# Aatrick/LightDiffusion

Hardware: AMD Instinct MI355X
Metric: UNet denoise steps/sec at 512x512 (higher is better)
Workload: dtype f16 (fp32 accumulate); 1 GPU; SD1.5 512x512 UNet CFG step, euler_ancestral / normal-30, batch 8/GPU (UNet batch 16), latent 64x64; global_batch=8, parallelism=dp1 (replicas, RCCL cond broadcast), hip_graph=True, setup_before_warmup=hipGraph capture + one untimed schedule pass per workload

## Files before the change

### include/ld_mi355x.h

```cpp
#ifndef LD_MI355X_H
#define LD_MI355X_H

#include <stddef.h>
#include <stdint.h>

#ifdef __cplusplus
extern "C" {
#endif

#define LD_OK 0
#define LD_ERR_ARG 1
#define LD_ERR_SHAPE 2
#define LD_ERR_HIP 3
#define LD_ERR_STATE 4

#define LD_F16 0
#define LD_F32 1

const char* ld_version(void);
const char* ld_status_string(int status);

typedef struct {
    int in_channels, out_channels, model_channels;
    int num_levels;
// ... 59 lines not shown

typedef struct {
    int in_nc, out_nc;
    int nf, gc;
    int nb;
    int scale;
} ld_esrgan_config;

typedef struct ld_esrgan ld_esrgan;

int ld_esrgan_create(const ld_esrgan_config* cfg, ld_esrgan** out);
void ld_esrgan_destroy(ld_esrgan* e);
int ld_esrgan_param_count(const ld_esrgan* e);
int ld_esrgan_param_info(const ld_esrgan* e, int index, const char** name, int* ndim, int64_t shape[4]);
int ld_esrgan_load_param(ld_esrgan* e, const char* name, const void* dev_src, int dtype, void* stream);
int ld_esrgan_reserve(ld_esrgan* e, int max_b, int max_h, int max_w);
size_t ld_esrgan_workspace_bytes(const ld_esrgan* e);
size_t ld_esrgan_plan_bytes(ld_esrgan* e, int b, int h, int w);
int ld_esrgan_forward(ld_esrgan* e, const float* x, float* out, int b, int h, int w, void* stream);
int ld_esrgan_profile(ld_esrgan* e, const float* x, float* out, int b, int h, int w, void* stream);
int ld_esrgan_profile_launches(const ld_esrgan* e, char* buf, size_t buf_bytes);
int ld_esrgan_last_launches(const ld_esrgan* e);
double ld_esrgan_last_flops(const ld_esrgan* e);

int ld_op_linear(const void* x, const void* w, const void* bias, const void* residual, void* y, int M, int N, int K,
                 float alpha, int act, void* ws, size_t ws_bytes, void* stream);
int ld_op_conv(const void* x1, int c1, const void* x2, int c2, int n, int h, int w, int hv, int wv, int stride, int ksize,
               const void* wt, const void* bias, const void* rowvec, const void* residual, void* y, int cout,
               void* ws, size_t ws_bytes, void* stream);
size_t ld_op_groupnorm_conv_ws_bytes(int c1, int c2, int n, int h, int w, int cout);
int ld_op_groupnorm_conv(const void* x1, int c1, const void* x2, int c2, int n, int h, int w, const void* gamma, const void* beta, float eps,
                         const void* wt, const void* bias, const void* rowvec, const void* residual, void* y, int cout, void* ws,
                         size_t ws_bytes, void* stream);
int ld_op_repack_conv(const void* src_oihw, int dtype, int cout, int cin, void* dst, void* stream);
size_t ld_op_conv_skip_ws_bytes(int c, int sc1, int sc2, int cout);
int ld_op_conv_skip(const void* x, int c, int n, int h, int w, const void* wt, const void* bias, const void* s1, int sc1, const void* s2, int sc2,
                    const void* wskip, const void* bskip, const void* rowvec, void* y, int cout, void* ws, size_t ws_bytes, void* stream);
size_t ld_op_groupnorm_conv_skip_ws_bytes(int c, int sc1, int sc2, int cout, int n, int h, int w);
int ld_op_groupnorm_conv_skip(const void* x, int c, int n, int h, int w, const void* gamma, const void* beta, float eps, const void* wt, const void* bias,
                              const void* s1, int sc1, const void* s2, int sc2, const void* wskip, const void* bskip, const void* rowvec, void* y, int cout,
                              float* part, int* chunks, void* ws, size_t ws_bytes, void* stream);
int ld_op_upconv2x_fold(const void* wt, int cout, int cin, void* wfold, void* stream);
int ld_op_upconv2x(const void* x, int c, int n, int h, int w, int hv, int wv, const void* wt, const void* wfold, const void* bias, void* y, int cout,
                   void* ws, size_t ws_bytes, void* stream);
size_t ld_op_conv_gn_partials_floats(int n, int hw);
int ld_op_conv_gn_partials(const void* x, int c, int n, int h, int w, int hv, int wv, const void* wt, const void* bias,
                           const void* residual, void* y, int cout, float* part, int* chunks, void* ws, size_t ws_bytes, void* stream);
size_t ld_op_groupnorm_ws_bytes(int n, int hw);
int ld_op_groupnorm(const void* x1, int c1, const void* x2, int c2, int n, int hw, const void* gamma, const void* beta,
                    float eps, int silu, void* y, void* ws, void* stream);
int ld_op_layernorm(const void* x, const void* gamma, const void* beta, void* y, int rows, int c, float eps, void* stream);
int ld_op_attention(const void* q, int ldq, const void* k, int ldk, const void* vt, int ldvt, void* o, int ldo, int b,
                    int heads, int lq, int lk, int d, float scale, int causal, void* stream);
int ld_op_attention_rowv(const void* q, int ldq, const void* k, int ldk, const void* v, int ldv, void* o, int ldo, int b,
                         int heads, int lq, int lk, int d, float scale, int causal, void* stream);
int ld_op_softmax_rows(void* s, int rows, int cols, void* stream);
int ld_op_timestep_embed(const float* sigma, const float* log_sigmas, int n_sigmas, int n, int dim, void* out_f16, float* t_out,
                         void* stream);
int ld_op_cfg_combine(const float* den2, float* out, float cfg, size_t n_half, void* stream);
int ld_op_axpby(float* x, float a, const float* y, float b, const float* z, float c, size_t n, void* stream);
int ld_op_hook_check(const void* a, const void* b, size_t words_ab, const void* x, size_t half_words_x, const void* sigma, int half_sigma,
                     int* flags, int epoch, void* stream);

int ld_op_linear_ln(const void* x, const void* w_prod, const void* b_prod, const void* gamma, const void* beta, const void* w,
                    const void* bias, void* t_out, void* y, int M, int C, int N, float eps, void* ws, size_t ws_bytes, void* stream);
int ld_op_linear_ln_geglu(const void* x, const void* w_prod, const void* b_prod, const void* gamma, const void* beta, const void* w,
                          const void* bias, void* t_out, void* y, int M, int C, int N, float eps, void* ws, size_t ws_bytes, void* stream);
int ld_op_bislerp(const float* x, float* tmp, float* y, int n, int c, int h, int w, int h_new, int w_new, void* stream);
int ld_op_esrgan_conv(const void* x, int ldx, int cin, int n, int h, int w, int up, const void* wt, const void* bias, void* y, int ldy, int c_off, int cout,
                      float slope, const void* r1, int ldr1, float s1, const void* r2, int ldr2, float s2, void* stream);
int ld_op_tile_blend(const float* ps, const float* my, const float* mx, int th, int tw, float* out, float* div, int oh, int ow, int y0, int x0, int c,
                     void* stream);
const char* ld_op_last_kernel(void);
int ld_op_lora_merge(const void* base_f16, void* dst_f16, int rows, int cols, const ld_lora_term* terms, int n_terms, void* stream);

int ld_op_u8_resample(const void* src, int src_pitch, int in_w, int in_h, int channels, void* dst, int dst_pitch, int out_w, int out_h, const int* hcoef,
                      int hk, const int* vcoef, int vk, void* tmp, void* stream);
size_t ld_op_u8_resample_tmp_bytes(int in_h, int out_w, int channels);
int ld_op_u8_box_weights(float radius, int* box_radius, unsigned* ww, unsigned* fw);
size_t ld_op_u8_blur_tmp_bytes(int w, int h);
int ld_op_u8_gaussian_blur(const void* src, int src_pitch, void* dst, int dst_pitch, int w, int h, float radius, void* tmp, void* stream);
int ld_op_u8_mask(void* dst, int dst_pitch, int w, int h, int px, int py, int pw, int ph, const void* pattern, int pattern_pitch, void* stream);
int ld_op_u8_composite(void* canvas, int canvas_pitch, int cw, int ch, const void* tile, int tile_pitch, const void* alpha, int alpha_pitch, int x0, int y0,
                       int w, int h, int channels, void* stream);
int ld_op_u8_from_f32(const float* x, void* y, size_t n, void* stream);
int ld_op_f32_from_u8(const void* x, float* y, size_t n, void* stream);

#ifdef __cplusplus
}
#endif
#endif
```

### lightdiffusion_amd/_lib.py

```python
from __future__ import annotations

import ctypes as C
import os

_HERE = os.path.dirname(os.path.abspath(__file__))
LIB_PATH = os.environ.get("LD_MI355X_LIB") or os.path.join(_HERE, "libld_mi355x.so")

OK, ERR_ARG, ERR_SHAPE, ERR_HIP, ERR_STATE = 0, 1, 2, 3, 4
F16, F32 = 0, 1


class UNetConfig(C.Structure):
    _fields_ = [("in_channels", C.c_int), ("out_channels", C.c_int), ("model_channels", C.c_int), ("num_levels", C.c_int),
                ("channel_mult", C.c_int * 8), ("num_res_blocks", C.c_int * 8), ("transformer_depth", C.c_int * 16),
                ("transformer_depth_output", C.c_int * 24), ("transformer_depth_middle", C.c_int),
                ("context_dim", C.c_int), ("num_heads", C.c_int)]


class VAEConfig(C.Structure):
    _fields_ = [("z_channels", C.c_int), ("ch", C.c_int), ("num_levels", C.c_int), ("ch_mult", C.c_int * 8),
                ("num_res_blocks", C.c_int), ("out_ch", C.c_int), ("with_encoder", C.c_int)]


class ESRGANConfig(C.Structure):
# ... 31 lines not shown
    "ld_unet_profile_pair": (_I, [_P, _P, _P, _P, _I, _I, _I, _P, C.POINTER(C.c_double), C.POINTER(C.c_double), C.POINTER(_I)]),
    "ld_unet_profile": (_I, [_P, _P, _P, _P, _I, _I, _I, _P, C.POINTER(C.c_double), C.POINTER(C.c_double), C.POINTER(_I)]),
    "ld_unet_profile_kernels": (_I, [_P, C.c_char_p, _Z]),
    "ld_unet_profile_launches": (_I, [_P, C.c_char_p, _Z]),
    "ld_unet_patch_param": (_I, [_P, C.c_char_p, C.POINTER(LoraTerm), _I, _P]),
    "ld_unet_unpatch": (_I, [_P, C.c_char_p, _P]),
    "ld_unet_read_param": (_I, [_P, C.c_char_p, _P, _P]),
    "ld_unet_refresh_derived": (_I, [_P, _P]),
    "ld_unet_patch_bytes": (_Z, [_P]),
    "ld_unet_last_launches": (_I, [_P]),
    "ld_unet_last_flops": (C.c_double, [_P]),
    "ld_vae_create": (_I, [C.POINTER(VAEConfig), C.POINTER(_P)]),
    "ld_vae_destroy": (None, [_P]),
    "ld_vae_param_count": (_I, [_P]),
    "ld_vae_param_info": (_I, [_P, _I, C.POINTER(C.c_char_p), C.POINTER(_I), C.POINTER(C.c_int64)]),
    "ld_vae_load_param": (_I, [_P, C.c_char_p, _P, _I, _P]),
    "ld_vae_reserve": (_I, [_P, _I, _I, _I]),
    "ld_vae_workspace_bytes": (_Z, [_P]),
    "ld_vae_plan_bytes": (_Z, [_P, _I, _I, _I]),
    "ld_vae_decode": (_I, [_P, _P, _P, _I, _I, _I, _P]),
    "ld_vae_encode": (_I, [_P, _P, _P, _I, _I, _I, _P]),
    "ld_vae_profile": (_I, [_P, _P, _P, _I, _I, _I, _P]),
    "ld_vae_profile_launches": (_I, [_P, C.c_char_p, _Z]),
    "ld_vae_last_launches": (_I, [_P]),
    "ld_vae_last_flops": (C.c_double, [_P]),
    "ld_esrgan_create": (_I, [C.POINTER(ESRGANConfig), C.POINTER(_P)]),
    "ld_esrgan_destroy": (None, [_P]),
    "ld_esrgan_param_count": (_I, [_P]),
    "ld_esrgan_param_info": (_I, [_P, _I, C.POINTER(C.c_char_p), C.POINTER(_I), C.POINTER(C.c_int64)]),
    "ld_esrgan_load_param": (_I, [_P, C.c_char_p, _P, _I, _P]),
    "ld_esrgan_reserve": (_I, [_P, _I, _I, _I]),
    "ld_esrgan_workspace_bytes": (_Z, [_P]),
    "ld_esrgan_plan_bytes": (_Z, [_P, _I, _I, _I]),
    "ld_esrgan_forward": (_I, [_P, _P, _P, _I, _I, _I, _P]),
    "ld_esrgan_profile": (_I, [_P, _P, _P, _I, _I, _I, _P]),
    "ld_esrgan_profile_launches": (_I, [_P, C.c_char_p, _Z]),
    "ld_esrgan_last_launches": (_I, [_P]),
    "ld_esrgan_last_flops": (C.c_double, [_P]),
    "ld_op_linear": (_I, [_P, _P, _P, _P, _P, _I, _I, _I, _F, _I, _P, _Z, _P]),
    "ld_op_conv": (_I, [_P, _I, _P, _I, _I, _I, _I, _I, _I, _I, _I, _P, _P, _P, _P, _P, _I, _P, _Z, _P]),
    "ld_op_groupnorm_conv_ws_bytes": (_Z, [_I, _I, _I, _I, _I, _I]),
    "ld_op_groupnorm_conv": (_I, [_P, _I, _P, _I, _I, _I, _I, _P, _P, _F, _P, _P, _P, _P, _P, _I, _P, _Z, _P]),
    "ld_op_repack_conv": (_I, [_P, _I, _I, _I, _P, _P]),
    "ld_op_upconv2x_fold": (_I, [_P, _I, _I, _P, _P]),
    "ld_op_upconv2x": (_I, [_P, _I, _I, _I, _I, _I, _I, _P, _P, _P, _P, _I, _P, _Z, _P]),
    "ld_op_conv_skip_ws_bytes": (_Z, [_I, _I, _I, _I]),
    "ld_op_conv_skip": (_I, [_P, _I, _I, _I, _I, _P, _P, _P, _I, _P, _I, _P, _P, _P, _P, _I, _P, _Z, _P]),
    "ld_op_groupnorm_conv_skip_ws_bytes": (_Z, [_I, _I, _I, _I, _I, _I, _I]),
    "ld_op_groupnorm_conv_skip": (_I, [_P, _I, _I, _I, _I, _P, _P, _F, _P, _P, _P, _I, _P, _I, _P, _P, _P, _P, _I, _P, _P, _P, _Z, _P]),
    "ld_op_groupnorm_ws_bytes": (_Z, [_I, _I]),
    "ld_op_groupnorm": (_I, [_P, _I, _P, _I, _I, _I, _P, _P, _F, _I, _P, _P, _P]),
    "ld_op_layernorm": (_I, [_P, _P, _P, _P, _I, _I, _F, _P]),
    "ld_op_attention": (_I, [_P, _I, _P, _I, _P, _I, _P, _I, _I, _I, _I, _I, _I, _F, _I, _P]),
    "ld_op_conv_gn_partials_floats": (_Z, [_I, _I]),
    "ld_op_conv_gn_partials": (_I, [_P, _I, _I, _I, _I, _I, _I, _P, _P, _P, _P, _I, _P, _P, _P, _Z, _P]),
    "ld_op_attention_rowv": (_I, [_P, _I, _P, _I, _P, _I, _P, _I, _I, _I, _I, _I, _I, _F, _I, _P]),
    "ld_op_softmax_rows": (_I, [_P, _I, _I, _P]),
    "ld_op_timestep_embed": (_I, [_P, _P, _I, _I, _I, _P, _P, _P]),
    "ld_op_cfg_combine": (_I, [_P, _P, _F, _Z, _P]),
    "ld_op_axpby": (_I, [_P, _F, _P, _F, _P, _F, _Z, _P]),
    "ld_op_hook_check": (_I, [_P, _P, _Z, _P, _Z, _P, _I, _P, _I, _P]),
    "ld_op_linear_ln": (_I, [_P, _P, _P, _P, _P, _P, _P, _P, _P, _I, _I, _I, _F, _P, _Z, _P]),
    "ld_op_linear_ln_geglu": (_I, [_P, _P, _P, _P, _P, _P, _P, _P, _P, _I, _I, _I, _F, _P, _Z, _P]),
    "ld_op_bislerp": (_I, [_P, _P, _P, _I, _I, _I, _I, _I, _I, _P]),
    "ld_op_esrgan_conv": (_I, [_P, _I, _I, _I, _I, _I, _I, _P, _P, _P, _I, _I, _I, _F, _P, _I, _F, _P, _I, _F, _P]),
    "ld_op_tile_blend": (_I, [_P, _P, _P, _I, _I, _P, _P, _I, _I, _I, _I, _I, _P]),
    "ld_op_last_kernel": (C.c_char_p, []),
    "ld_op_lora_merge": (_I, [_P, _P, _I, _I, C.POINTER(LoraTerm), _I, _P]),
    "ld_op_u8_resample": (_I, [_P, _I, _I, _I, _I, _P, _I, _I, _I, _P, _I, _P, _I, _P, _P]),
    "ld_op_u8_resample_tmp_bytes": (_Z, [_I, _I, _I]),
    "ld_op_u8_box_weights": (_I, [_F, C.POINTER(_I), C.POINTER(C.c_uint), C.POINTER(C.c_uint)]),
    "ld_op_u8_blur_tmp_bytes": (_Z, [_I, _I]),
    "ld_op_u8_gaussian_blur": (_I, [_P, _I, _P, _I, _I, _I, _F, _P, _P]),
    "ld_op_u8_mask": (_I, [_P, _I, _I, _I, _I, _I, _I, _I, _P, _I, _P]),
    "ld_op_u8_composite": (_I, [_P, _I, _I, _I, _P, _I, _P, _I, _I, _I, _I, _I, _I, _P]),
    "ld_op_u8_from_f32": (_I, [_P, _P, _Z, _P]),
    "ld_op_f32_from_u8": (_I, [_P, _P, _Z, _P]),
}


def lib() -> C.CDLL:
    global _lib
    if _lib is None:
        if not os.path.exists(LIB_PATH):
            raise ImportError(f"{LIB_PATH} not found — build it with `python -c 'import __graft_entry__ as g; g.build()'` "
                              f"or `make -C lightdiffusion_amd/csrc`.  There is no CPU / PyTorch fallback for the hot path.")
        try:
            import torch
        except ImportError:
            pass
        l = C.CDLL(LIB_PATH)
        missing = []
        for name, (res, args) in SIGNATURES.items():
            if not hasattr(l, name):
                if not os.environ.get("LD_MI355X_LIB"):
                    raise AttributeError(f"{LIB_PATH} does not export {name}: header and library out of sync — rebuild it")
                missing.append(name)
                setattr(l, name, _missing_symbol(name))
                continue
            fn = getattr(l, name)
            fn.restype = res
            fn.argtypes = args
        l._ld_missing = tuple(missing)
        _lib = l
    return _lib

# ... 11 lines not shown
```

### lightdiffusion_amd/csrc/attention.hip

```cpp
#include <cstdlib>
#include <type_traits>

#include <string>

#include "kernels.h"

namespace {

constexpr int AT_THREADS = 256;

__device__ uint4 g_att_zero[8];
__device__ uint4 g_att_ones = {0x3C003C00u, 0x3C003C00u, 0x3C003C00u, 0x3C003C00u};
__device__ uint4 g_att_one_last = {0u, 0u, 0u, 0x3C000000u};
typedef __fp16 fp16x4_t __attribute__((__vector_size__(4 * sizeof(__fp16))));
typedef _Float16 half4v __attribute__((ext_vector_type(4)));

template <int DK, bool MASKED, int NW, int WPS, bool VROW>
__global__ __launch_bounds__(64 * NW, WPS) void flash_attn2_kernel(const AttnParams p) {
    constexpr int DV = (DK + 1) / 2;
    constexpr bool ONES = (DK & 1) != 0;
    constexpr int KT = 64;
    constexpr int NT2 = 64 * NW;
    constexpr int LIT = (DV * 256 + NT2 - 1) / NT2;
    constexpr int TILE_CH = LIT * NT2;
// ... 436 lines not shown
        else hipLaunchKernelGGL((flash_attn2_kernel<DK, false, 8, W8, VROW>), dim3((unsigned)nblk8), dim3(512), 0, s, p);
    } else {
        if (masked) hipLaunchKernelGGL((flash_attn2_kernel<DK, true, 4, AUTO_WPS, VROW>), dim3(nblk), dim3(AT_THREADS), 0, s, p);
        else hipLaunchKernelGGL((flash_attn2_kernel<DK, false, 4, AUTO_WPS, VROW>), dim3(nblk), dim3(AT_THREADS), 0, s, p);
    }
}

template <int D>
void launch_attn512(const AttnParams& p, hipStream_t s) {
    const int nblk = ((p.Lq + 127) / 128) * p.B;
    const bool masked = p.causal || (p.Lk % 32) != 0;
    static const std::string names[2] = {"flash_attn512_kernel<" + std::to_string(D) + ",plain>", "flash_attn512_kernel<" + std::to_string(D) + ",masked>"};
    t_last_attn_kernel = names[masked ? 1 : 0].c_str();
    if (masked) hipLaunchKernelGGL((flash_attn512_kernel<D, true>), dim3(nblk), dim3(512), 0, s, p);
    else hipLaunchKernelGGL((flash_attn512_kernel<D, false>), dim3(nblk), dim3(512), 0, s, p);
}

}

const char* attention_last_kernel_name() { return t_last_attn_kernel; }

int attention_launch(const AttnParams& p, hipStream_t stream) {
    t_last_attn_kernel = "";
    if (p.Q == nullptr || p.K == nullptr || (p.Vt == nullptr) == (p.V == nullptr) || p.O == nullptr) return LD_ERR_ARG;
    if (p.B <= 0 || p.H <= 0 || p.Lq <= 0 || p.Lk <= 0) return LD_ERR_SHAPE;
    if (p.d % 8 || p.d <= 0 || (p.d > 160 && !((p.d == 512 || p.d == 256) && p.H == 1 && p.V != nullptr))) return LD_ERR_SHAPE;
    if ((p.ldq & 7) || (p.ldk & 7) || (p.ldo & 3) || (p.sQ & 7) || (p.sK & 7) || (p.sV & 7)) return LD_ERR_SHAPE;
    const long long hd = (long long)p.H * p.d;
    if (p.ldq < hd || p.ldk < hd || p.ldo < hd) return LD_ERR_SHAPE;
    if (p.B > 1 && (p.sQ < (long long)(p.Lq - 1) * p.ldq + hd || p.sK < (long long)(p.Lk - 1) * p.ldk + hd || p.sO < (long long)(p.Lq - 1) * p.ldo + hd)) return LD_ERR_SHAPE;
    const int dk = (p.d + 15) / 16;
    if (p.V != nullptr) {
        if ((p.ldv & 7) || p.ldv < hd) return LD_ERR_SHAPE;
        if (p.B > 1 && p.sV < (long long)(p.Lk - 1) * p.ldv + hd) return LD_ERR_SHAPE;
        if (p.d == 512 || p.d == 256) {
            if (p.d == 512) launch_attn512<512>(p, stream);
            else launch_attn512<256>(p, stream);
            return hipGetLastError() == hipSuccess ? LD_OK : LD_ERR_HIP;
        }
        switch (dk) {
            case 1: launch_attn<1, true>(p, stream); break;
            case 2: launch_attn<2, true>(p, stream); break;
            case 3: launch_attn<3, true>(p, stream); break;
            case 4: launch_attn<4, true>(p, stream); break;
            case 5: launch_attn<5, true>(p, stream); break;
            case 6: launch_attn<6, true>(p, stream); break;
            case 8: launch_attn<8, true>(p, stream); break;
            case 10: launch_attn<10, true>(p, stream); break;
            default: return LD_ERR_SHAPE;
        }
        return hipGetLastError() == hipSuccess ? LD_OK : LD_ERR_HIP;
    }
    if ((p.ldvt & 7) || p.ldvt < ((p.Lk + 7) & ~7)) return LD_ERR_SHAPE;
    switch (dk) {
        case 1: launch_attn<1, false>(p, stream); break;
        case 2: launch_attn<2, false>(p, stream); break;
        case 3: launch_attn<3, false>(p, stream); break;
        case 4: launch_attn<4, false>(p, stream); break;
        case 5: launch_attn<5, false>(p, stream); break;
        case 6: launch_attn<6, false>(p, stream); break;
        case 8: launch_attn<8, false>(p, stream); break;
        case 10: launch_attn<10, false>(p, stream); break;
        default: return LD_ERR_SHAPE;
    }
    return hipGetLastError() == hipSuccess ? LD_OK : LD_ERR_HIP;
}
```

### lightdiffusion_amd/csrc/capi.hip

```cpp
#include <string>

#include "kernels.h"
#include "../../include/ld_mi355x.h"

namespace {
inline size_t align256(size_t v) { return (v + 255) / 256 * 256; }

thread_local std::string t_op_kernels;
inline void op_begin() { t_op_kernels.clear(); }
inline int noted(int st, const char* name) {
    if (name != nullptr && *name != '\0') {
        if (!t_op_kernels.empty()) t_op_kernels += ';';
        t_op_kernels += name;
    }
    return st;
}
inline int gemm_op(const GemmParams& p, hipStream_t s) { return noted(gemm_launch(p, s), gemm_last_kernel_name()); }
inline int gemm_op(const GemmParams& p, const GemmPlan& plan, hipStream_t s) { return noted(gemm_run(p, plan, s), gemm_last_kernel_name()); }

constexpr size_t kSyncBytes = LD_SYNC_INTS * sizeof(int);
inline size_t conv8_scratch_head(int cout, int cin) { return kSyncBytes + (conv8_weight_eligible(cout, cin) ? align256(conv8_weight_bytes(cout, cin)) : 0); }
inline void conv8_scratch(GemmParams& p, void* ws, size_t partial_bytes) {
    const int cin = p.C1 + p.C2;
    p.sync = (int*)ws;
// ... 248 lines not shown
size_t ld_op_groupnorm_conv_skip_ws_bytes(int c, int sc1, int sc2, int cout, int n, int h, int w) {
    op_begin();
    const size_t HW = (size_t)h * w;
    return ld_op_conv_skip_ws_bytes(c, sc1, sc2, cout) + align256(groupnorm_workspace_bytes(n, (int)HW)) + 2 * align256((size_t)n * c * sizeof(float)) +
           align256((size_t)n * HW * c * sizeof(half_t));
}

int ld_op_groupnorm_conv_skip(const void* x, int c, int n, int h, int w, const void* gamma, const void* beta, float eps, const void* wt, const void* bias,
                              const void* s1, int sc1, const void* s2, int sc2, const void* wskip, const void* bskip, const void* rowvec, void* y, int cout,
                              float* part, int* chunks, void* ws, size_t ws_bytes, void* stream_) {
    op_begin();
    if (x == nullptr || wt == nullptr || bias == nullptr || s1 == nullptr || wskip == nullptr || bskip == nullptr || y == nullptr || ws == nullptr) return LD_ERR_ARG;
    if (c <= 0 || sc1 <= 0 || sc2 < 0 || (sc2 > 0 && s2 == nullptr) || cout <= 0 || n <= 0 || h <= 0 || w <= 0) return LD_ERR_ARG;
    if ((gamma == nullptr) != (beta == nullptr) || (part == nullptr) != (chunks == nullptr)) return LD_ERR_ARG;
    if (ws_bytes < ld_op_groupnorm_conv_skip_ws_bytes(c, sc1, sc2, cout, n, h, w)) return LD_ERR_ARG;
    if (chunks != nullptr) *chunks = 0;
    return op_conv_skip(x, c, n, h, w, wt, bias, s1, sc1, s2, sc2, wskip, bskip, rowvec, gamma, beta, eps, y, cout, part, chunks, (char*)ws, (hipStream_t)stream_);
}

int ld_op_repack_conv(const void* src, int dtype, int cout, int cin, void* dst, void* stream) {
    op_begin();
    return repack_conv3x3_launch(src, dtype == LD_F32, cout, cin, (half_t*)dst, (hipStream_t)stream);
}

size_t ld_op_groupnorm_ws_bytes(int n, int hw) {
    op_begin();
    return groupnorm_workspace_bytes(n, hw);
}

int ld_op_groupnorm(const void* x1, int c1, const void* x2, int c2, int n, int hw, const void* gamma, const void* beta, float eps,
                    int silu, void* y, void* ws, void* stream) {
    op_begin();
    return groupnorm_launch((const half_t*)x1, c1, (const half_t*)x2, c2, n, hw, (const half_t*)gamma, (const half_t*)beta, eps,
                            silu, (half_t*)y, (float*)ws, (hipStream_t)stream);
}

int ld_op_layernorm(const void* x, const void* gamma, const void* beta, void* y, int rows, int c, float eps, void* stream) {
    op_begin();
    return layernorm_launch((const half_t*)x, (const half_t*)gamma, (const half_t*)beta, (half_t*)y, rows, c, eps, (hipStream_t)stream);
}

int ld_op_attention(const void* q, int ldq, const void* k, int ldk, const void* vt, int ldvt, void* o, int ldo, int b, int heads,
                    int lq, int lk, int d, float scale, int causal, void* stream) {
    op_begin();
    AttnParams a;
    a.Q = (const half_t*)q; a.ldq = ldq; a.sQ = (long long)lq * ldq;
    a.K = (const half_t*)k; a.ldk = ldk; a.sK = (long long)lk * ldk;
    a.Vt = (const half_t*)vt; a.ldvt = ldvt; a.sV = (long long)heads * d * ldvt;
    a.O = (half_t*)o; a.ldo = ldo; a.sO = (long long)lq * ldo;
    a.B = b; a.H = heads; a.Lq = lq; a.Lk = lk; a.d = d; a.scale = scale; a.causal = causal;
    return attn_op(a, (hipStream_t)stream);
}

int ld_op_attention_rowv(const void* q, int ldq, const void* k, int ldk, const void* v, int ldv, void* o, int ldo, int b, int heads,
                         int lq, int lk, int d, float scale, int causal, void* stream) {
    op_begin();
    const char *qb = (const char*)q, *kb = (const char*)k, *vb = (const char*)v;
    const long long rowb = (long long)ldq * 2;
    const bool fused = ldq == ldk && ldk == ldv && rowb > 0 && (kb - qb >= 0 ? kb - qb : qb - kb) < rowb && (vb - qb >= 0 ? vb - qb : qb - vb) < rowb;
    if (fused && lq != lk) return LD_ERR_SHAPE;
    AttnParams a;
    a.Q = (const half_t*)q; a.ldq = ldq; a.sQ = (long long)lq * ldq;
    a.K = (const half_t*)k; a.ldk = ldk; a.sK = (long long)lk * ldk;
    a.V = (const half_t*)v; a.ldv = ldv; a.sV = (long long)lk * ldv;
    a.O = (half_t*)o; a.ldo = ldo; a.sO = (long long)lq * ldo;
    a.B = b; a.H = heads; a.Lq = lq; a.Lk = lk; a.d = d; a.scale = scale; a.causal = causal;
    return attn_op(a, (hipStream_t)stream);
}

int ld_op_softmax_rows(void* s, int rows, int cols, void* stream) {
    op_begin();
    return softmax_rows_launch((half_t*)s, rows, cols, cols, (hipStream_t)stream);
}

int ld_op_timestep_embed(const float* sigma, const float* log_sigmas, int n_sigmas, int n, int dim, void* out, float* t_out, void* stream) {
    op_begin();
    return timestep_embed_launch(sigma, log_sigmas, n_sigmas, n, dim, (half_t*)out, t_out, (hipStream_t)stream);
}

int ld_op_cfg_combine(const float* den2, float* out, float cfg, size_t n_half, void* stream) {
    op_begin();
    return cfg_combine_launch(den2, out, cfg, n_half, (hipStream_t)stream);
}

int ld_op_hook_check(const void* a, const void* b, size_t words_ab, const void* x, size_t half_words_x, const void* sigma, int half_sigma,
                     int* flags, int epoch, void* stream) {
    op_begin();
    return hook_check_launch(a, b, words_ab, x, half_words_x, sigma, half_sigma, flags, epoch, (hipStream_t)stream);
}

int ld_op_axpby(float* x, float a, const float* y, float b, const float* z, float c, size_t n, void* stream) {
    op_begin();
    return axpby_launch(x, a, y, b, z, c, n, (hipStream_t)stream);
}

int ld_op_linear_ln(const void* x, const void* w_prod, const void* b_prod, const void* gamma, const void* beta, const void* w,
                    const void* bias, void* t_out, void* y, int M, int C, int N, float eps, void* ws, size_t ws_bytes, void* stream_) {
    op_begin();
    if (x == nullptr || w_prod == nullptr || gamma == nullptr || beta == nullptr || w == nullptr || t_out == nullptr || y == nullptr ||
        ws == nullptr)
        return LD_ERR_ARG;
    hipStream_t stream = (hipStream_t)stream_;
    const size_t wb = align256((size_t)N * C * sizeof(half_t)), bb = align256((size_t)N * sizeof(half_t)), sb = align256((size_t)N * sizeof(float));
    const size_t stb = align256((size_t)((C + 63) / 64) * M * 2 * sizeof(float));
    if (ws_bytes < wb + bb + sb + stb) return LD_ERR_ARG;
    char* wsp = (char*)ws;
// ... 162 lines not shown
```

### lightdiffusion_amd/csrc/kernels.h

```cpp
#pragma once
#include <cstdint>
#include <cstdlib>
#include "common.h"
#include "gemm.h"

static inline int gn_num_chunks(int n_img, int HW) {
    const long long px = (long long)(n_img < 1 ? 1 : n_img) * HW;
    const int target = px <= 8192 ? 512 : (px <= 131072 ? 1024 : 2048);
    int p = target / (4 * (n_img < 1 ? 1 : n_img));
    if (p > HW / 8) p = HW / 8;
    if (p > 256) p = 256;
    return p < 1 ? 1 : p;
}
size_t groupnorm_workspace_bytes(int n_img, int HW);
int groupnorm_launch(const half_t* x1, int C1, const half_t* x2, int C2, int n_img, int HW, const half_t* gamma,
                     const half_t* beta, float eps, int silu, half_t* y, float* partial, hipStream_t stream, int stats_ready = 0);
int groupnorm_stats_launch(const half_t* x1, int C1, const half_t* x2, int C2, int n_img, int HW, float* partial, hipStream_t stream);
int groupnorm_scale_shift_launch(const half_t* x1, int C1, const half_t* x2, int C2, int n_img, int HW, const half_t* gamma, const half_t* beta,
                                 float eps, float* partial, float* scale, float* shift, hipStream_t stream, int stats_ready = 0);
int layernorm_launch(const half_t* x, const half_t* gamma, const half_t* beta, half_t* y, int rows, int C, float eps,
                     hipStream_t stream);
int softmax_rows_launch(half_t* s, int rows, int cols, long long ld, hipStream_t stream, int valid = 0);

struct AttnParams {
    const half_t* Q = nullptr;
    const half_t* K = nullptr;
    const half_t* Vt = nullptr;
    const half_t* V = nullptr;
    int ldv = 0;
    half_t* O = nullptr;
    int ldq = 0, ldk = 0, ldvt = 0, ldo = 0;
    long long sQ = 0, sK = 0, sV = 0, sO = 0;
    int B = 0, H = 0, Lq = 0, Lk = 0, d = 0;
    float scale = 1.0f;
    int causal = 0;
};
int attention_launch(const AttnParams& p, hipStream_t stream);
const char* attention_last_kernel_name();

int ln_fold_launch(const half_t* W, int N, int K, const half_t* gamma, const half_t* beta, const half_t* bias, half_t* Wout, half_t* bout,
                   float* wsum, hipStream_t stream);
int mlp_out_fold_launch(const half_t* Wpo, const half_t* W2, const half_t* b2, const half_t* bpo, int C, half_t* Wout, half_t* bout, hipStream_t stream);
int skip_fold_launch(const half_t* W2, const half_t* Wsk, const half_t* b2, const half_t* bsk, int N, int K9, int SC, half_t* Wout, half_t* bout,
                     hipStream_t stream);
int upconv_fold_launch(const half_t* W, int O, int I, half_t* Wout, hipStream_t stream);
struct SmallConvInArgs {
    const float* x = nullptr;
    const float* scale_sigma = nullptr;
    const half_t* pre_w = nullptr;
    const half_t* pre_b = nullptr;
    const half_t* w = nullptr;
    const half_t* b = nullptr;
    half_t* y = nullptr;
    int N = 0, Cin = 0, H = 0, W = 0, Cout = 0;
    long long dup_off = 0;
};
int small_conv_in_launch(const SmallConvInArgs& a, hipStream_t stream);

struct SmallConvOutArgs {
    const half_t* x = nullptr;
    const half_t* w = nullptr;
    const half_t* b = nullptr;
    int N = 0, H = 0, W = 0, Cin = 0, Cout = 0;
    int mode = 0;
    const float* x_in = nullptr;
    const float* sigma = nullptr;
    float* out = nullptr;
    int in_mod = 0;
};
int small_conv_out_launch(const SmallConvOutArgs& a, hipStream_t stream);

int vae_out_finish_launch(const half_t* t8, float* out, long long npix, int cout, hipStream_t stream);

int small_pointwise_launch(const half_t* x, const half_t* w, const half_t* b, float* out, int N, int HW, int C, hipStream_t stream);

int timestep_embed_launch(const float* sigma, const float* log_sigmas, int n_sig, int N, int dim, half_t* out, float* t_out,
                          hipStream_t stream, int sigma_mod = 0);

struct DupArgs {
    char* base[3] = {nullptr, nullptr, nullptr};
    unsigned long long bytes[3] = {0, 0, 0};
    int count = 0;
};
int dup_halves_launch(const DupArgs& a, hipStream_t stream);

int repack_conv3x3_launch(const void* src, int src_is_f32, int O, int I, half_t* dst, hipStream_t stream);
int repack_rows_launch(const void* src, int src_is_f32, int rows, int cols, half_t* dst, int geglu_bn, hipStream_t stream);
int ctx_pad_launch(const void* src, int src_is_f32, int n, int T, int Tp, int D, half_t* dst, hipStream_t stream);
int fill_half_launch(half_t* dst, size_t n, float v, hipStream_t stream);

// ... 65 lines not shown
```

### lightdiffusion_amd/csrc/unet.hip

```cpp
#include <cstring>

#include "runtime.h"
#include "../../include/ld_mi355x.h"

namespace {

struct ResW {
    std::string prefix;
    int cin = 0, cout = 0, emb_off = 0;
    int gn1_g, gn1_b, c1_w, c1_b, emb_w, emb_b, gn2_g, gn2_b, c2_w, c2_b, sk_w = -1, sk_b = -1;
    size_t f_c2_w = 0, f_c2_b = 0;
};
struct StW {
    int c = 0, bn = 0, ctx_slot = 0;
    size_t f_qk_w = 0, f_q2_w = 0, f_ff1_w = 0, f_qk_b = 0, f_q2_b = 0, f_ff1_b = 0, f_qk_s = 0, f_q2_s = 0,
           f_ff1_s = 0;
    size_t f_mo_w = 0, f_mo_b = 0;
    int gn_g, gn_b, pin_w, pin_b, ln1_g, ln1_b, q1_w, k1_w, v1_w, o1_w, o1_b, ln2_g, ln2_b, q2_w, k2_w, v2_w, o2_w, o2_b, ln3_g,
        ln3_b, ff1_w, ff1_b, ff2_w, ff2_b, pout_w, pout_b;
};
struct ConvW {
    int cin = 0, cout = 0, w = -1, b = -1;
    long long f_up = -1;
};
// ... 404 lines not shown
            p.W = reinterpret_cast<const half_t*>(fb + s.f_qk_w); p.ldw = C;
            p.M = M; p.N = 3 * C; p.K = C;
            p.C = qkv; p.ldc = 3 * C;
            p.bias_n = reinterpret_cast<const half_t*>(fb + s.f_qk_b);
            ln_args(p, s.f_qk_s);
            ex.gemm(p);
        }
        {
            AttnParams a;
            a.Q = qkv; a.ldq = 3 * C; a.sQ = (long long)L * 3 * C;
            a.K = qkv + C; a.ldk = 3 * C; a.sK = (long long)L * 3 * C;
            a.V = qkv + 2 * C; a.ldv = 3 * C; a.sV = (long long)L * 3 * C;
            a.O = ao; a.ldo = C; a.sO = (long long)L * C;
            a.B = n; a.H = heads; a.Lq = L; a.Lk = L; a.d = d;
            a.scale = 1.0f / sqrtf((float)d);
            ex.attention(a);
        }
        const bool split_here = pair_pending;
        producer(ao, C, s.o1_w, s.o1_b, t, C);
        half_t* q2 = qkv;
        {
            GemmParams p;
            p.A = t; p.lda = C;
            p.W = reinterpret_cast<const half_t*>(fb + s.f_q2_w); p.ldw = C;
            p.M = M; p.N = C; p.K = C;
            p.C = q2; p.ldc = C;
            p.bias_n = reinterpret_cast<const half_t*>(fb + s.f_q2_b);
            ln_args(p, s.f_q2_s);
            ex.gemm(p);
        }
        if (split_here) {
            const size_t hb = (size_t)M * C * sizeof(half_t);
            DupArgs da;
            da.count = 3;
            da.base[0] = reinterpret_cast<char*>(t); da.base[1] = reinterpret_cast<char*>(q2); da.base[2] = reinterpret_cast<char*>(const_cast<half_t*>(x));
            da.bytes[0] = da.bytes[1] = da.bytes[2] = hb;
            ex.launches += 1;
            ex.t_begin(KC_MISC, 0.0, 1, "dup3", (long long)hb, 0, 0, 1);
            if (!ex.dry && ex.status == LD_OK) ex.note(dup_halves_launch(da, ex.stream));
            ex.t_end("dup_halves_kernel");
            pair_pending = false;
            n = n_alloc;
            M = n * L;
        }
        {
            const int Tp = u->ctx_tpad;
            AttnParams a;
            a.Q = q2; a.ldq = C; a.sQ = (long long)L * C;
            a.K = u->ctx_k[s.ctx_slot]; a.ldk = C; a.sK = (long long)Tp * C;
            a.Vt = u->ctx_vt[s.ctx_slot]; a.ldvt = Tp; a.sV = (long long)C * Tp;
            a.O = ao; a.ldo = C; a.sO = (long long)L * C;
            a.B = n; a.H = heads; a.Lq = L; a.Lk = u->ctx_tok; a.d = d;
            a.scale = 1.0f / sqrtf((float)d);
            ex.attention(a);
        }
        producer(ao, C, s.o2_w, s.o2_b, t, C);
        ff = ar.halfs(Ma * 4 * C);
        {
            GemmParams p;
            p.A = t; p.lda = C;
            p.W = reinterpret_cast<const half_t*>(fb + s.f_ff1_w); p.ldw = C;
            p.M = M; p.N = 8 * C; p.K = C;
            p.bias_n = reinterpret_cast<const half_t*>(fb + s.f_ff1_b);
            p.act = 2; p.bn = s.bn;
            p.C = ff; p.ldc = 4 * C; p.ldr = 4 * C;
            ln_args(p, s.f_ff1_s);
            ex.gemm(p);
        }
        {
            GemmParams p;
            p.conv = 1; p.ksize = 1;
            p.A = ff; p.A2 = t; p.C1 = 4 * C; p.C2 = C;
            p.Hs = p.Hv = p.Ho = H; p.Ws = p.Wv = p.Wo = W; p.stride = 1;
            p.W = reinterpret_cast<const half_t*>(fb + s.f_mo_w); p.ldw = 5 * C;
            p.M = M; p.N = C; p.K = 5 * C;
            p.bias_n = reinterpret_cast<const half_t*>(fb + s.f_mo_b);
            p.R = x; p.ldr = C;
            p.C = out; p.ldc = C;
            want_stats(p, gno, L, &gno_done);
            ex.gemm(p);
        }
        ar.release(mk);
        return {out, C, H, W, gno_done ? gno : nullptr, gno_done};
    }
};

int fold_layernorms(ld_unet* u, hipStream_t stream) {
    for (const StW& s : u->st) {
        const int C = s.c;
        char* fb = u->fold_base;
        auto H = [&](size_t off) { return reinterpret_cast<half_t*>(fb + off); };
        auto F = [&](size_t off) { return reinterpret_cast<float*>(fb + off); };
        const half_t* P_q1 = u->pt.ptr(s.q1_w);
        int st = ln_fold_launch(P_q1, 3 * C, C, u->pt.ptr(s.ln1_g), u->pt.ptr(s.ln1_b), nullptr, H(s.f_qk_w), H(s.f_qk_b), F(s.f_qk_s), stream);
        if (st == LD_OK) st = ln_fold_launch(u->pt.ptr(s.q2_w), C, C, u->pt.ptr(s.ln2_g), u->pt.ptr(s.ln2_b), nullptr, H(s.f_q2_w), H(s.f_q2_b), F(s.f_q2_s), stream);
        if (st == LD_OK) st = ln_fold_launch(u->pt.ptr(s.ff1_w), 8 * C, C, u->pt.ptr(s.ln3_g), u->pt.ptr(s.ln3_b), u->pt.ptr(s.ff1_b), H(s.f_ff1_w), H(s.f_ff1_b), F(s.f_ff1_s), stream);
        if (st == LD_OK) st = mlp_out_fold_launch(u->pt.ptr(s.pout_w), u->pt.ptr(s.ff2_w), u->pt.ptr(s.ff2_b), u->pt.ptr(s.pout_b), C, H(s.f_mo_w), H(s.f_mo_b), stream);
        if (st != LD_OK) return st;
    }
    for (const ResW& r : u->res) {
        if (r.sk_w < 0) continue;
        const int st = skip_fold_launch(u->pt.ptr(r.c2_w), u->pt.ptr(r.sk_w), u->pt.ptr(r.c2_b), u->pt.ptr(r.sk_b), r.cout, 9 * r.cout, r.cin,
                                        reinterpret_cast<half_t*>(u->fold_base + r.f_c2_w), reinterpret_cast<half_t*>(u->fold_base + r.f_c2_b), stream);
        if (st != LD_OK) return st;
    }
    for (const ConvW& c : u->convs) {
// ... 515 lines not shown
```

### lightdiffusion_amd/ops.py

```python
from __future__ import annotations

import math
from typing import Optional

import torch

from ._lib import F16, F32, check, lib


def _stream() -> int:
    return torch.cuda.current_stream().cuda_stream


def _p(t: Optional[torch.Tensor]) -> Optional[int]:
    if t is None:
        return None
    assert t.is_cuda and t.is_contiguous(), "device-resident contiguous tensors only"
    return t.data_ptr()


def last_kernel() -> str:
    return lib().ld_op_last_kernel().decode()


# ... 140 lines not shown
    y = torch.empty(n, hv, wv, cout, dtype=torch.float16, device=x.device)
    part = torch.zeros(lib().ld_op_conv_gn_partials_floats(n, hv * wv), dtype=torch.float32, device=x.device)
    chunks = ctypes.c_int(0)
    ws = _ws(192 << 20, x.device)
    check(lib().ld_op_conv_gn_partials(_p(x), c, n, h, w, hv, wv, _p(w_packed), _p(bias), _p(residual), _p(y), cout, _p(part), ctypes.byref(chunks),
                                       _p(ws), ws.numel(), _stream()), "ld_op_conv_gn_partials")
    if chunks.value == 0:
        return y, None
    return y, part[: n * chunks.value * 64].view(n, chunks.value, 32, 2)


def group_norm_silu_conv2d(x: torch.Tensor, gamma: torch.Tensor, beta: torch.Tensor, eps: float, w_packed: torch.Tensor,
                           bias: Optional[torch.Tensor], x2: Optional[torch.Tensor] = None, rowvec: Optional[torch.Tensor] = None,
                           residual: Optional[torch.Tensor] = None) -> torch.Tensor:
    n, h, w, c1 = x.shape
    c2 = 0 if x2 is None else x2.shape[-1]
    cout = w_packed.shape[0]
    y = torch.empty(n, h, w, cout, dtype=torch.float16, device=x.device)
    ws = _ws(lib().ld_op_groupnorm_conv_ws_bytes(c1, c2, n, h, w, cout), x.device)
    check(lib().ld_op_groupnorm_conv(_p(x), c1, _p(x2), c2, n, h, w, _p(gamma), _p(beta), eps, _p(w_packed), _p(bias), _p(rowvec), _p(residual),
                                     _p(y), cout, _p(ws), ws.numel(), _stream()), "ld_op_groupnorm_conv")
    return y


def group_norm(x: torch.Tensor, gamma: torch.Tensor, beta: torch.Tensor, eps: float, silu: bool = False,
               x2: Optional[torch.Tensor] = None) -> torch.Tensor:
    n, c1 = x.shape[0], x.shape[-1]
    hw = x.numel() // (n * c1)
    c2 = 0 if x2 is None else x2.shape[-1]
    y = torch.empty(*x.shape[:-1], c1 + c2, dtype=torch.float16, device=x.device)
    ws = _ws(lib().ld_op_groupnorm_ws_bytes(n, hw), x.device)
    check(lib().ld_op_groupnorm(_p(x), c1, _p(x2), c2, n, hw, _p(gamma), _p(beta), eps, int(silu), _p(y), _p(ws), _stream()),
          "ld_op_groupnorm")
    return y


def layer_norm(x: torch.Tensor, gamma: torch.Tensor, beta: torch.Tensor, eps: float = 1e-5) -> torch.Tensor:
    c = x.shape[-1]
    y = torch.empty_like(x)
    check(lib().ld_op_layernorm(_p(x), _p(gamma), _p(beta), _p(y), x.numel() // c, c, eps, _stream()), "ld_op_layernorm")
    return y


def attention(q: torch.Tensor, k: torch.Tensor, v: torch.Tensor, heads: int, causal: bool = False) -> torch.Tensor:
    b, lq, c = q.shape
    lk = k.shape[1]
    d = c // heads
    lkp = (lk + 7) // 8 * 8
    vt = torch.zeros(b, c, lkp, dtype=torch.float16, device=q.device)
    vt[:, :, :lk] = v.transpose(1, 2)
    o = torch.empty_like(q)
    check(lib().ld_op_attention(_p(q), c, _p(k.contiguous()), c, _p(vt), lkp, _p(o), c, b, heads, lq, lk, d, 1.0 / math.sqrt(d), int(causal), _stream()),
          "ld_op_attention")
    return o


def attention_qkv(qkv: torch.Tensor, heads: int, causal: bool = False) -> torch.Tensor:
    b, l, c3 = qkv.shape
    c = c3 // 3
    d = c // heads
    o = torch.empty(b, l, c, dtype=torch.float16, device=qkv.device)
    base = qkv.data_ptr()
    check(lib().ld_op_attention_rowv(base, c3, base + 2 * c, c3, base + 4 * c, c3, _p(o), c, b, heads, l, l, d, 1.0 / math.sqrt(d), int(causal),
                                     _stream()), "ld_op_attention_rowv")
    return o


def attention_rowv(q: torch.Tensor, k: torch.Tensor, v: torch.Tensor, heads: int, causal: bool = False) -> torch.Tensor:
    b, lq, c = q.shape
    lk = k.shape[1]
    d = c // heads
    o = torch.empty_like(q)
    check(lib().ld_op_attention_rowv(_p(q), c, _p(k.contiguous()), c, _p(v.contiguous()), c, _p(o), c, b, heads, lq, lk, d, 1.0 / math.sqrt(d), int(causal),
                                     _stream()), "ld_op_attention_rowv")
    return o


def softmax_rows_(s: torch.Tensor) -> torch.Tensor:
    cols = s.shape[-1]
    check(lib().ld_op_softmax_rows(_p(s), s.numel() // cols, cols, _stream()), "ld_op_softmax_rows")
    return s


def timestep_embed(sigma: torch.Tensor, log_sigmas: torch.Tensor, dim: int):
    n = sigma.numel()
    out = torch.empty(n, dim, dtype=torch.float16, device=sigma.device)
    t = torch.empty(n, dtype=torch.float32, device=sigma.device)
    check(lib().ld_op_timestep_embed(_p(sigma), _p(log_sigmas), log_sigmas.numel(), n, dim, _p(out), _p(t), _stream()),
          "ld_op_timestep_embed")
    return out, t


def cfg_combine(den2: torch.Tensor, cfg: float) -> torch.Tensor:
    half = den2.shape[0] // 2
    out = torch.empty_like(den2[:half])
    check(lib().ld_op_cfg_combine(_p(den2), _p(out), float(cfg), out.numel(), _stream()), "ld_op_cfg_combine")
    return out


def axpby_(x: torch.Tensor, a: float, y: Optional[torch.Tensor] = None, b: float = 0.0, z: Optional[torch.Tensor] = None,
           c: float = 0.0) -> torch.Tensor:
    check(lib().ld_op_axpby(_p(x), float(a), _p(y), float(b), _p(z), float(c), x.numel(), _stream()), "ld_op_axpby")
    return x


def bislerp(samples: torch.Tensor, width: int, height: int) -> torch.Tensor:
# ... 253 lines not shown
```

Baseline: 64.53 steps/s.

## Add specialized cross-attention kernel with LDS-resident K/V for short contexts

Adds a dedicated cross-attention kernel for context lengths up to 96 keys that loads the whole K and V^T for a (batch, head) into LDS once and processes many 32-row query blocks per workgroup with MFMA. It uses a single-pass softmax with no online rescaling, and head dims 40/80/160 get an implicit ones-column for the row sum. The UNet cross-attention call sites opt in through a kv_resident flag, and a new C API entry is exposed. The aim is to cut redundant K/V reloads and flash-loop overhead in the 77-token cross-attention. The cost is another specialized code path with swizzle and tail-masking complexity.

```diff
diff --git a/include/ld_mi355x.h b/include/ld_mi355x.h
--- a/include/ld_mi355x.h
+++ b/include/ld_mi355x.h
@@ -135,6 +135,8 @@
 int ld_op_layernorm(const void* x, const void* gamma, const void* beta, void* y, int rows, int c, float eps, void* stream);
 int ld_op_attention(const void* q, int ldq, const void* k, int ldk, const void* vt, int ldvt, void* o, int ldo, int b,
                     int heads, int lq, int lk, int d, float scale, int causal, void* stream);
+int ld_op_attention_ctx(const void* q, int ldq, const void* k, int ldk, const void* vt, int ldvt, void* o, int ldo, int b,
+                        int heads, int lq, int lk, int d, float scale, int causal, void* stream);
 int ld_op_attention_rowv(const void* q, int ldq, const void* k, int ldk, const void* v, int ldv, void* o, int ldo, int b,
                          int heads, int lq, int lk, int d, float scale, int causal, void* stream);
 int ld_op_softmax_rows(void* s, int rows, int cols, void* stream);
diff --git a/lightdiffusion_amd/_lib.py b/lightdiffusion_amd/_lib.py
--- a/lightdiffusion_amd/_lib.py
+++ b/lightdiffusion_amd/_lib.py
@@ -107,6 +107,7 @@
     "ld_op_groupnorm": (_I, [_P, _I, _P, _I, _I, _I, _P, _P, _F, _I, _P, _P, _P]),
     "ld_op_layernorm": (_I, [_P, _P, _P, _P, _I, _I, _F, _P]),
     "ld_op_attention": (_I, [_P, _I, _P, _I, _P, _I, _P, _I, _I, _I, _I, _I, _I, _F, _I, _P]),
+    "ld_op_attention_ctx": (_I, [_P, _I, _P, _I, _P, _I, _P, _I, _I, _I, _I, _I, _I, _F, _I, _P]),
     "ld_op_conv_gn_partials_floats": (_Z, [_I, _I]),
     "ld_op_conv_gn_partials": (_I, [_P, _I, _I, _I, _I, _I, _I, _P, _P, _P, _P, _I, _P, _P, _P, _Z, _P]),
     "ld_op_attention_rowv": (_I, [_P, _I, _P, _I, _P, _I, _P, _I, _I, _I, _I, _I, _I, _F, _I, _P]),
diff --git a/lightdiffusion_amd/csrc/attention.hip b/lightdiffusion_amd/csrc/attention.hip
--- a/lightdiffusion_amd/csrc/attention.hip
+++ b/lightdiffusion_amd/csrc/attention.hip
@@ -512,6 +512,10 @@
         return hipGetLastError() == hipSuccess ? LD_OK : LD_ERR_HIP;
     }
     if ((p.ldvt & 7) || p.ldvt < ((p.Lk + 7) & ~7)) return LD_ERR_SHAPE;
+    if (p.kv_resident) {
+        if (xattn_resident_contract(p)) return xattn_resident_launch(p, stream, &t_last_attn_kernel);
+        if (p.kv_resident > 1) return LD_ERR_SHAPE;
+    }
     switch (dk) {
         case 1: launch_attn<1, false>(p, stream); break;
         case 2: launch_attn<2, false>(p, stream); break;
diff --git a/lightdiffusion_amd/csrc/capi.hip b/lightdiffusion_amd/csrc/capi.hip
--- a/lightdiffusion_amd/csrc/capi.hip
+++ b/lightdiffusion_amd/csrc/capi.hip
@@ -324,6 +324,19 @@
     return attn_op(a, (hipStream_t)stream);
 }
 
+int ld_op_attention_ctx(const void* q, int ldq, const void* k, int ldk, const void* vt, int ldvt, void* o, int ldo, int b, int heads,
+                        int lq, int lk, int d, float scale, int causal, void* stream) {
+    op_begin();
+    AttnParams a;
+    a.Q = (const half_t*)q; a.ldq = ldq; a.sQ = (long long)lq * ldq;
+    a.K = (const half_t*)k; a.ldk = ldk; a.sK = (long long)lk * ldk;
+    a.Vt = (const half_t*)vt; a.ldvt = ldvt; a.sV = (long long)heads * d * ldvt;
+    a.O = (half_t*)o; a.ldo = ldo; a.sO = (long long)lq * ldo;
+    a.B = b; a.H = heads; a.Lq = lq; a.Lk = lk; a.d = d; a.scale = scale; a.causal = causal;
+    a.kv_resident = 2;
+    return attn_op(a, (hipStream_t)stream);
+}
+
 int ld_op_attention_rowv(const void* q, int ldq, const void* k, int ldk, const void* v, int ldv, void* o, int ldo, int b, int heads,
                          int lq, int lk, int d, float scale, int causal, void* stream) {
     op_begin();
diff --git a/lightdiffusion_amd/csrc/kernels.h b/lightdiffusion_amd/csrc/kernels.h
--- a/lightdiffusion_amd/csrc/kernels.h
+++ b/lightdiffusion_amd/csrc/kernels.h
@@ -34,8 +34,11 @@
     int B = 0, H = 0, Lq = 0, Lk = 0, d = 0;
     float scale = 1.0f;
     int causal = 0;
+    int kv_resident = 0;
 };
 int attention_launch(const AttnParams& p, hipStream_t stream);
+bool xattn_resident_contract(const AttnParams& p);
+int xattn_resident_launch(const AttnParams& p, hipStream_t stream, const char** name);
 const char* attention_last_kernel_name();
 
 int ln_fold_launch(const half_t* W, int N, int K, const half_t* gamma, const half_t* beta, const half_t* bias, half_t* Wout, half_t* bout,
diff --git a/lightdiffusion_amd/csrc/unet.hip b/lightdiffusion_amd/csrc/unet.hip
--- a/lightdiffusion_amd/csrc/unet.hip
+++ b/lightdiffusion_amd/csrc/unet.hip
@@ -480,6 +480,7 @@
             a.O = ao; a.ldo = C; a.sO = (long long)L * C;
             a.B = n; a.H = heads; a.Lq = L; a.Lk = u->ctx_tok; a.d = d;
             a.scale = 1.0f / sqrtf((float)d);
+            a.kv_resident = 1;
             ex.attention(a);
         }
         producer(ao, C, s.o2_w, s.o2_b, t, C);
diff --git a/lightdiffusion_amd/csrc/xattn.hip b/lightdiffusion_amd/csrc/xattn.hip
--- /dev/null
+++ b/lightdiffusion_amd/csrc/xattn.hip
@@ -0,0 +1,252 @@
+#include <string>
+#include <type_traits>
+
+#include "kernels.h"
+
+namespace {
+
+__device__ uint4 g_xa_zero;
+__device__ uint4 g_xa_ones = {0x3C003C00u, 0x3C003C00u, 0x3C003C00u, 0x3C003C00u};
+
+constexpr int XA_KEYS = 96;
+
+template <int DK, int NW, int WPS>
+__global__ __launch_bounds__(64 * NW, WPS) void xattn_resident_kernel(const AttnParams p, const int S) {
+    constexpr int DV = (DK + 1) / 2;
+    constexpr bool ONES = (DK & 1) != 0;
+    constexpr int NT = 64 * NW;
+    constexpr int LITK = (2 * XA_KEYS * DK + NT - 1) / NT;
+    constexpr int LITV = (3 * 128 * DV + NT - 1) / NT;
+    constexpr int KCH = LITK * NT, VCH = LITV * NT;
+    constexpr int SUBV = 128 * DV * 8;
+    __shared__ __attribute__((aligned(16))) half_t smem[(KCH + VCH) * 8];
+
+    const int tid = threadIdx.x, lane = tid & 63;
+    const int wid = __builtin_amdgcn_readfirstlane(tid >> 6);
+    const int r = lane & 31, hh = lane >> 5;
+    int bid = xcd_remap(blockIdx.x, p.B * p.H * S);
+    const int head = bid % p.H;
+    bid /= p.H;
+    const int seg = bid % S, b = bid / S;
+    const int d = p.d, dch = d >> 3;
+    const int nb = (p.Lq + 31) >> 5;
+    const int blk0 = (int)((long long)seg * nb / S), blk1 = (int)((long long)(seg + 1) * nb / S);
+
+    const half_t* Qg = p.Q + (long long)b * p.sQ + head * d + 8 * hh;
+    const half_t* Kg = p.K + (long long)b * p.sK + head * d;
+    const half_t* Vg = p.Vt + (long long)b * p.sV + (long long)head * d * p.ldvt;
+    const half_t* zp = reinterpret_cast<const half_t*>(&g_xa_zero);
+    const half_t* op = reinterpret_cast<const half_t*>(&g_xa_ones);
+
+    auto qload = [&](int blk, uint4 (&q)[DK]) {
+        const int row = blk * 32 + r;
+        const half_t* src = Qg + (long long)row * p.ldq;
+#pragma unroll
+        for (int ks = 0; ks < DK; ++ks) q[ks] = (row < p.Lq && 16 * ks + 8 * hh < d) ? ld16(src + 16 * ks) : zero16();
+    };
+    int blk = blk0 + wid;
+    uint4 qn[DK];
+#pragma unroll
+    for (int ks = 0; ks < DK; ++ks) qn[ks] = zero16();
+    if (blk < blk1) qload(blk, qn);
+
+    int tz = 0;
+    while (tz < 3 && !((dch >> tz) & 1)) ++tz;
+    const int sw_mask = (1 << tz) - 1, sw_shift = 3 - tz;
+
+    const unsigned smem_base = __builtin_amdgcn_readfirstlane(lds_addr(smem)) + (unsigned)(wid * 64) * 16u;
+    auto vslot = [&](int i, const half_t*& src, int& nv, bool& ones) {
+        const int q = tid + i * NT;
+        const int sub = q / (128 * DV), rem = q - sub * (128 * DV);
+        const int vr = rem >> 2, key0 = (sub * 4 + ((rem & 3) ^ ((vr >> 2) & 3))) << 3;
+        src = Vg + (long long)vr * p.ldvt + key0;
+        nv = (q < 3 * 128 * DV && vr < d) ? p.Lk - key0 : 0;
+        ones = ONES && q < 3 * 128 * DV && vr == 32 * DV - 1;
+    };
+    uint4 fix[LITV];
+#pragma unroll
+    for (int i = 0; i < LITV; ++i) {
+        const half_t* src;
+        int nv;
+        bool ones;
+        vslot(i, src, nv, ones);
+        fix[i] = (nv > 0 && nv < 8) ? ld16(src) : zero16();
+    }
+#pragma unroll
+    for (int i = 0; i < LITV; ++i) {
+        const half_t* src;
+        int nv;
+        bool ones;
+        vslot(i, src, nv, ones);
+        glds16(nv >= 8 ? src : (ones ? op : zp), smem_base + (unsigned)(KCH + i * NT) * 16u);
+    }
+#pragma unroll
+    for (int i = 0; i < LITK; ++i) {
+        const int q = tid + i * NT;
+        const int row = q / dch, cph = q - row * dch;
+        const int key = (row & ~12) | ((row & 4) << 1) | ((row & 8) >> 1);
+        const bool data = row < XA_KEYS && key < p.Lk;
+        glds16(data ? Kg + (long long)key * p.ldk + ((cph ^ ((row >> sw_shift) & sw_mask)) << 3) : zp, smem_base + (unsigned)(i * NT) * 16u);
+    }
+    wait_vmcnt<0>();
+#pragma unroll
+    for (int i = 0; i < LITV; ++i) {
+        const half_t* src;
+        int nv;
+        bool ones;
+        vslot(i, src, nv, ones);
+        if (nv > 0 && nv < 8) {
+            const unsigned w[4] = {fix[i].x, fix[i].y, fix[i].z, fix[i].w};
+            unsigned m[4];
+#pragma unroll
+            for (int j = 0; j < 4; ++j) m[j] = 2 * j + 1 < nv ? w[j] : (2 * j < nv ? (w[j] & 0xFFFFu) : 0u);
+            st16(smem + (size_t)(KCH + tid + i * NT) * 8, make_uint4(m[0], m[1], m[2], m[3]));
+        }
+    }
+    __syncthreads();
+
+    const int ksw = (r >> sw_shift) & sw_mask;
+    int koff[DK];
+#pragma unroll
+    for (int ks = 0; ks < DK; ++ks) koff[ks] = (r * dch + ((2 * ks + hh) ^ ksw)) << 3;
+    int voff[2];
+#pragma unroll
+    for (int k2 = 0; k2 < 2; ++k2) voff[k2] = KCH * 8 + ((r * 4 + ((2 * k2 + hh) ^ ((r >> 2) & 3))) << 3);
+
+    const int nsub = (p.Lk + 31) >> 5;
+    const int tail = p.Lk - (nsub - 1) * 32;
+    const float c2 = p.scale * 1.44269504088896340736f;
+
+    auto run = [&](auto nsc) {
+        constexpr int NS = decltype(nsc)::value;
+        for (; blk < blk1; blk += NW) {
+            asm volatile("" ::: "memory");
+            half8 qf[DK];
+#pragma unroll
+            for (int ks = 0; ks < DK; ++ks) {
+                float qv[8];
+                unpack8(qn[ks], qv);
+#pragma unroll
+                for (int j = 0; j < 8; ++j) qv[j] *= c2;
+                qf[ks] = as_half8(pack8(qv));
+            }
+            if (blk + NW < blk1) qload(blk + NW, qn);
+
+            f32x16 s[NS];
+#pragma unroll
+            for (int sub = 0; sub < NS; ++sub) {
+#pragma unroll
+                for (int e = 0; e < 16; ++e) s[sub][e] = 0.f;
+#pragma unroll
+                for (int ks = 0; ks < DK; ++ks) {
+                    const half8 kf = as_half8(ld16(smem + sub * 32 * d + koff[ks]));
+                    s[sub] = __builtin_amdgcn_mfma_f32_32x32x16_f16(kf, qf[ks], s[sub], 0, 0, 0);
+                }
+            }
+            if (tail < 32) {
+#pragma unroll
+                for (int e = 0; e < 16; ++e) {
+                    const int i = (e & 3) + 8 * (e >> 2) + 4 * hh;
+                    const int key = (i & ~12) | ((i & 4) << 1) | ((i & 8) >> 1);
+                    if (key >= tail) s[NS - 1][e] = -INFINITY;
+                }
+            }
+            float mx = fmaxf(fmaxf(s[0][0], s[0][1]), s[0][2]);
+#pragma unroll
+            for (int e = 3; e + 1 < 16; e += 2) mx = fmaxf(fmaxf(mx, s[0][e]), s[0][e + 1]);
+            mx = fmaxf(mx, s[0][15]);
+#pragma unroll
+            for (int sub = 1; sub < NS; ++sub)
+#pragma unroll
+                for (int e = 0; e < 16; e += 2) mx = fmaxf(fmaxf(mx, s[sub][e]), s[sub][e + 1]);
+            {
+                const auto sw = __builtin_amdgcn_permlane32_swap(__float_as_uint(mx), __float_as_uint(mx), false, false);
+                mx = fmaxf(__uint_as_float(sw[0]), __uint_as_float(sw[1]));
+            }
+            float psum = 0.f;
+            half8 pf[NS][2];
+#pragma unroll
+            for (int sub = 0; sub < NS; ++sub)
+#pragma unroll
+                for (int e = 0; e < 16; e += 2) {
+                    const float p0 = __builtin_amdgcn_exp2f(s[sub][e] - mx);
+                    const float p1 = __builtin_amdgcn_exp2f(s[sub][e + 1] - mx);
+                    if (!ONES) psum += p0 + p1;
+                    const half2v h2 = __builtin_bit_cast(half2v, pk2h(p0, p1));
+                    pf[sub][e >> 3][e & 7] = h2[0];
+                    pf[sub][e >> 3][(e & 7) + 1] = h2[1];
+                }
+            f32x16 o[DV];
+#pragma unroll
+            for (int tt = 0; tt < DV; ++tt) {
+#pragma unroll
+                for (int e = 0; e < 16; ++e) o[tt][e] = 0.f;
+#pragma unroll
+                for (int sub = 0; sub < NS; ++sub)
+#pragma unroll
+                    for (int k2 = 0; k2 < 2; ++k2) {
+                        const half8 vf = as_half8(ld16(smem + sub * SUBV + tt * 1024 + voff[k2]));
+                        o[tt] = __builtin_amdgcn_mfma_f32_32x32x16_f16(vf, pf[sub][k2], o[tt], 0, 0, 0);
+                    }
+            }
+            float l_tot;
+            if (ONES) l_tot = __shfl(o[DV - 1][15], 32 + r, 64);
+            else l_tot = psum + __shfl_xor(psum, 32, 64);
+            const float inv = 1.0f / l_tot;
+            const int qrow = blk * 32 + r;
+            if (qrow < p.Lq) {
+                half_t* Og = p.O + (long long)b * p.sO + (long long)qrow * p.ldo + head * d;
+#pragma unroll
+                for (int tt = 0; tt < DV; ++tt)
+#pragma unroll
+                    for (int g = 0; g < 4; ++g) {
+                        const int dd = tt * 32 + 8 * g + 4 * hh;
+                        if (dd < d) {
+                            half4 h;
+#pragma unroll
+                            for (int e = 0; e < 4; ++e) h[e] = (half_t)(o[tt][4 * g + e] * inv);
+                            *reinterpret_cast<half4*>(Og + dd) = h;
+                        }
+                    }
+            }
+        }
+    };
+    if (nsub == 3) run(std::integral_constant<int, 3>{});
+    else if (nsub == 2) run(std::integral_constant<int, 2>{});
+    else run(std::integral_constant<int, 1>{});
+}
+
+template <int DK>
+constexpr int xa_wps() { return DK <= 3 ? 4 : (DK <= 5 ? 3 : 2); }
+
+template <int DK>
+int launch_xattn(const AttnParams& p, hipStream_t s, const char** name) {
+    constexpr int NW = 4, WPS = xa_wps<DK>();
+    static const std::string nm = "xattn_resident_kernel<" + std::to_string(DK) + "," + std::to_string(NW) + ">";
+    *name = nm.c_str();
+    const long long BH = (long long)p.B * p.H;
+    const int nb = (p.Lq + 31) / 32, steps = (nb + NW - 1) / NW;
+    const long long target = BH >= 256LL * WPS ? 1 : (256LL * WPS + BH - 1) / BH;
+    const long long two = steps / 2 > 1 ? steps / 2 : 1;
+    long long S = target < two ? target : two;
+    if (BH * S < 256) S = target < steps ? target : steps;
+    if (BH * S > 0x7fffffffLL) return LD_ERR_SHAPE;
+    hipLaunchKernelGGL((xattn_resident_kernel<DK, NW, WPS>), dim3((unsigned)(BH * S)), dim3(64 * NW), 0, s, p, (int)S);
+    return hipGetLastError() == hipSuccess ? LD_OK : LD_ERR_HIP;
+}
+
+}
+
+bool xattn_resident_contract(const AttnParams& p) {
+    const int dk = (p.d + 15) / 16;
+    return p.Vt != nullptr && p.V == nullptr && !p.causal && p.Lk >= 1 && p.Lk <= XA_KEYS && p.d > 0 && p.d % 8 == 0 && (dk == 3 || dk == 5 || dk == 10);
+}
+
+int xattn_resident_launch(const AttnParams& p, hipStream_t stream, const char** name) {
+    if (!xattn_resident_contract(p)) return LD_ERR_SHAPE;
+    switch ((p.d + 15) / 16) {
+        case 3: return launch_xattn<3>(p, stream, name);
+        case 5: return launch_xattn<5>(p, stream, name);
+        default: return launch_xattn<10>(p, stream, name);
+    }
+}
diff --git a/lightdiffusion_amd/ops.py b/lightdiffusion_amd/ops.py
--- a/lightdiffusion_amd/ops.py
+++ b/lightdiffusion_amd/ops.py
@@ -216,6 +216,23 @@
     o = torch.empty_like(q)
     check(lib().ld_op_attention(_p(q), c, _p(k.contiguous()), c, _p(vt), lkp, _p(o), c, b, heads, lq, lk, d, 1.0 / math.sqrt(d), int(causal), _stream()),
           "ld_op_attention")
+    return o
+
+
+def attention_ctx(q: torch.Tensor, k: torch.Tensor, vt: torch.Tensor, heads: int, lk: int = None, causal: bool = False, ldq: int = None) -> torch.Tensor:
+    b, lq = q.shape[0], q.shape[1]
+    c = k.shape[2]
+    lk = k.shape[1] if lk is None else lk
+    d = c // heads
+    assert vt.is_contiguous() and k.is_contiguous() and vt.shape[:2] == (b, c)
+    if ldq is None:
+        q = q.contiguous()
+        ldq = c
+    else:
+        assert q.is_cuda and q.stride(1) == ldq and q.stride(2) == 1 and q.stride(0) == lq * ldq
+    o = torch.empty(b, lq, c, dtype=torch.float16, device=q.device)
+    check(lib().ld_op_attention_ctx(q.data_ptr(), ldq, _p(k), c, _p(vt), vt.shape[2], _p(o), c, b, heads, lq, lk, d, 1.0 / math.sqrt(d), int(causal), _stream()),
+          "ld_op_attention_ctx")
     return o
 
 
```

Measured after the change: 64.78 steps/s (median of 6 runs). Within noise of the previous version (+0.4%).
